# alphacep/vosk-tts

Measured on NVIDIA H100. Metric: audio samples/sec @22.05kHz, 128-phoneme utterance, higher is better.
Workload: dtype fp32 (flow/decoder convs + attention: bf16 hi+lo split x3 MMAs on wgmma, fp32 accumulate; rest fp32 FFMA)

## Files before the change

### vosk_tts_b200/csrc/conv_tc.cuh

```cuda
#pragma once
#include <type_traits>
#include <cuda.h>
#include <cuda_bf16.h>
#include <cuda_runtime.h>
#include <stdint.h>
#include "wgmma.cuh"

namespace vtts {

constexpr int TC_BM = 128;
constexpr int TC_BK = 64;
#ifndef VTTS_TC_AST64
#define VTTS_TC_AST64 3
#endif
#ifndef VTTS_TC_WST64
#define VTTS_TC_WST64 4
#endif
#ifndef VTTS_TC_AST128
#define VTTS_TC_AST128 3
#endif
#ifndef VTTS_TC_WST128
#define VTTS_TC_WST128 4
#endif
template <int BN> constexpr int tc_ast() { return BN == 64 ? VTTS_TC_AST64 : VTTS_TC_AST128; }
template <int BN> constexpr int tc_wst() { return BN == 64 ? VTTS_TC_WST64 : VTTS_TC_WST128; }
constexpr int TC_CWG = 2;
constexpr int TC_THREADS = TC_CWG * 128 + 32;
constexpr int TC_MAXP = 4;

enum : int { TCE_RELU = 1, TCE_GATE = 2 };

struct TcProblemBase {
  CUtensorMap a_hi, a_lo, w_hi, w_lo;
  __nv_bfloat16* p_mid;
  const float* bias;
  const float* cond;
  const float* res;
  float* y;
  __nv_bfloat16* p_hi;
  __nv_bfloat16* p_lo;
  int cond_ld, ldr, roff, ldy, yoff, ldp, poff;
  int Cin, Cout, k, dil, pad;
  int out_mul, out_add;
  int in_extra, out_seq_extra;
  int epi;
  float alpha, pl_slope;
  int split;
  int cl0;
};
struct TcProblem : TcProblemBase {
  CUtensorMap a_mid, w_mid;
};

struct TcBatchScalars {
  int n;
  int rmul;
  int tall;
  int a_bytes;
  int baseoff;
  int cn;
  int wpre;
  int np;
  int ast, wst;
  int dbgskip;
  int wmc;
  int persist;
  int gx, gy, gz;
  int split;
  int mixed;
  int nb;
  unsigned long long* dbg;
};
template <class PT, int MP = TC_MAXP>
struct TcBatchT : TcBatchScalars {
  PT p[MP];
};
using TcBatch = TcBatchT<TcProblem>;
template <int MP>
inline TcBatchT<TcProblemBase, MP> tc_lite(const TcBatch& tb) {
  TcBatchT<TcProblemBase, MP> l;
  static_cast<TcBatchScalars&>(l) = tb;
  for (int i = 0; i < MP; ++i) l.p[i] = tb.p[i];
  return l;
}
__device__ __forceinline__ unsigned long long gtimer() {
  unsigned long long t;
  asm volatile("mov.u64 %0, %globaltimer;" : "=l"(t));
  return t;
}
#define TC_STAMP(i) do { if (tb.dbg && blockIdx.x == 0 && blockIdx.y == 0 && blockIdx.z == 0) tb.dbg[i] = gtimer(); } while (0)

__device__ __forceinline__ void tma_load_2d(void* dst, const CUtensorMap* map, int c0, int c1, uint64_t* bar) {
  asm volatile(
      "cp.async.bulk.tensor.2d.shared::cluster.global.mbarrier::complete_tx::bytes [%0], [%1, {%3, %4}], [%2];" ::"r"(smem_u32(dst)),
      "l"(reinterpret_cast<uint64_t>(map)), "r"(smem_u32(bar)), "r"(c0), "r"(c1)
      : "memory");
}
__device__ __forceinline__ void tma_load_2d_mc(void* dst, const CUtensorMap* map, int c0, int c1, uint64_t* bar, uint16_t mask) {
  asm volatile(
      "cp.async.bulk.tensor.2d.shared::cluster.global.mbarrier::complete_tx::bytes.multicast::cluster [%0], [%1, {%3, %4}], [%2], %5;" ::"r"(
          smem_u32(dst)),
      "l"(reinterpret_cast<uint64_t>(map)), "r"(smem_u32(bar)), "r"(c0), "r"(c1), "h"(mask)
      : "memory");
}
__device__ __forceinline__ uint32_t cluster_rank() {
  uint32_t r;
  asm volatile("mov.u32 %0, %%cluster_ctarank;" : "=r"(r));
  return r;
}
__device__ __forceinline__ void mbar_arrive_remote(uint64_t* bar, uint32_t rank) {
  uint32_t ra;
  asm volatile("mapa.shared::cluster.u32 %0, %1, %2;" : "=r"(ra) : "r"(smem_u32(bar)), "r"(rank));
  asm volatile("mbarrier.arrive.release.cluster.shared::cluster.b64 _, [%0];" ::"r"(ra) : "memory");
}
__device__ __forceinline__ void tc_release(uint64_t* bar, int n) {
  if (n > 1) {
    for (int r = 0; r < n; ++r) mbar_arrive_remote(bar, (uint32_t)r);
  } else {
    mbar_arrive(bar);
  }
}


struct TcEpi {
  const float* bias;
  const float* cond;
  const float* res;
  float* y;
  __nv_bfloat16 *p_hi, *p_lo, *p_mid;
  int ldr, roff, ldy, yoff, ldp, poff;
  int ncol;
  float alpha, pl_slope;
  bool gate, relu, store;
};
template <class PT>
__device__ __forceinline__ TcEpi tc_epi(const PT& P, int b, int dbgskip) {
  TcEpi E;
  E.bias = P.bias;
  E.cond = P.cond ? P.cond + (long)b * P.cond_ld : nullptr;
  E.res = (dbgskip & 4) ? nullptr : P.res;
  E.y = P.y;
  E.p_hi = P.p_hi; E.p_lo = P.p_lo; E.p_mid = P.p_mid;
  E.ldr = P.ldr; E.roff = P.roff; E.ldy = P.ldy; E.yoff = P.yoff; E.ldp = P.ldp; E.poff = P.poff;
  E.gate = (P.epi & TCE_GATE) != 0;
  E.relu = (P.epi & TCE_RELU) != 0;
  E.ncol = E.gate ? P.Cout >> 1 : P.Cout;
  E.alpha = P.alpha; E.pl_slope = P.pl_slope;
  E.store = !(dbgskip & 1);
  return E;
}
struct TcEpiCol {
  int c, oc, nout;
  bool ok;
};
__device__ __forceinline__ TcEpiCol tc_epi_col(const TcEpi& E, int c, bool in_tile) {
  TcEpiCol k;
  k.c = c;
  k.oc = E.gate ? c >> 1 : c;
  k.ok = in_tile && k.oc < E.ncol;
  k.nout = E.gate ? 1 : min(2, E.ncol - k.oc);
  return k;
}
struct TcEpiIn {
  float b0, b1, c0, c1, r[2][2];
};
__device__ __forceinline__ TcEpiIn tc_epi_load(const TcEpi& E, const TcEpiCol& k, const long (&orow)[2], const bool (&rowok)[2]) {
  TcEpiIn in = {};
  if (!(k.ok && (rowok[0] || rowok[1]))) return in;
  const bool two = E.gate || k.nout > 1;
  in.b0 = E.bias[k.c];
  if (two) in.b1 = E.bias[k.c + 1];
  if (E.cond) {
    in.c0 = E.cond[k.c];
    if (two) in.c1 = E.cond[k.c + 1];
  }
  if (E.res) {
#pragma unroll
    for (int h = 0; h < 2; ++h) {
      if (!rowok[h]) continue;
      const float* rp = E.res + orow[h] * (long)E.ldr + E.roff + k.oc;
      if (k.nout == 2 && ((E.ldr | E.roff | k.oc) & 1) == 0) {
        const float2 q2 = *reinterpret_cast<const float2*>(rp);
        in.r[h][0] = q2.x; in.r[h][1] = q2.y;
      } else {
        in.r[h][0] = rp[0];
        if (k.nout > 1) in.r[h][1] = rp[1];
      }
    }
  }
  return in;
}
__device__ __forceinline__ void tc_epi_store(const TcEpi& E, const TcEpiCol& k, long orow, float b0, float b1, float c0, float c1,
                                             float r0, float r1, float v0, float v1) {
  const float bv0 = E.cond ? b0 + c0 : b0, bv1 = E.cond ? b1 + c1 : b1;
  float u[2];
  if (E.gate) {
    const float a = v0 + bv0, s = v1 + bv1;
    u[0] = tanhf(a) * (1.f / (1.f + expf(-s)));
    u[1] = 0.f;
  } else {
    u[0] = v0 + bv0;
    u[1] = k.nout > 1 ? v1 + bv1 : 0.f;
  }
#pragma unroll
  for (int e = 0; e < 2; ++e) {
    float q = u[e];
    if (E.relu) q = fmaxf(q, 0.f);
    u[e] = __fmul_rn(q, E.alpha);
  }
  if (E.res) {
    u[0] = __fadd_rn(u[0], r0);
    if (k.nout > 1) u[1] = __fadd_rn(u[1], r1);
  }
  if (!E.store) return;
  const int oc = k.oc, nout = k.nout;
  if (E.y) {
    float* yr = E.y + orow * (long)E.ldy + E.yoff + oc;
    if (nout == 2 && ((E.ldy | E.yoff | oc) & 1) == 0) {
      *reinterpret_cast<float2*>(yr) = make_float2(u[0], u[1]);
    } else {
      yr[0] = u[0];
      if (nout > 1) yr[1] = u[1];
    }
  }
  if (E.p_hi) {
    const long po = orow * (long)E.ldp + E.poff + oc;
    __nv_bfloat16 hb[2], mb[2], lb[2];
#pragma unroll
    for (int e = 0; e < 2; ++e) {
      float q = u[e];
      q = q > 0.f ? q : q * E.pl_slope;
      if (E.p_mid) split_bf16_3(q, hb[e], mb[e], lb[e]);
      else split_bf16(q, hb[e], lb[e]);
    }
    if (nout == 2 && ((E.ldp | E.poff | oc) & 1) == 0) {
      *reinterpret_cast<__nv_bfloat162*>(E.p_hi + po) = __halves2bfloat162(hb[0], hb[1]);
      *reinterpret_cast<__nv_bfloat162*>(E.p_lo + po) = __halves2bfloat162(lb[0], lb[1]);
      if (E.p_mid) *reinterpret_cast<__nv_bfloat162*>(E.p_mid + po) = __halves2bfloat162(mb[0], mb[1]);
    } else {
      E.p_hi[po] = hb[0]; E.p_lo[po] = lb[0];
      if (E.p_mid) E.p_mid[po] = mb[0];
      if (nout > 1) {
        E.p_hi[po + 1] = hb[1]; E.p_lo[po + 1] = lb[1];
        if (E.p_mid) E.p_mid[po + 1] = mb[1];
      }
    }
  }
}

template <int BN>
constexpr int tc_smem_bytes(int a_bytes, int np = 2, int ast = tc_ast<BN>(), int wst = tc_wst<BN>()) {
  return ast * np * a_bytes + wst * np * BN * TC_BK * 2 + 1024  + 256 ;
}
constexpr int TC_MAXST = 4;

struct TcTile {
  int pi;
  int b, co0, t0, sp;
  int s;
  int t0u;
  bool valid;
};

template <int BN, bool MIXED, class PT, int MP>
__device__ __forceinline__ void conv_tc_body(const TcBatchT<PT, MP>& tb, const int* __restrict__ lens, const int* __restrict__ offs) {
  constexpr bool HAS_MID = std::is_same<PT, TcProblem>::value;
  constexpr int B_BYTES = BN * TC_BK * 2;
  constexpr int NACC = BN / 2;
  const int TC_AST = tb.ast, TC_WST = tb.wst, NP = HAS_MID ? tb.np : 2;
  PDL_LAUNCH();
  if (threadIdx.x == 0) TC_STAMP(0);
  const int S = tb.split;
  const bool persist = tb.persist != 0;
  const int A_BYTES = tb.a_bytes;
  const bool tall = tb.tall != 0;
  const int wmc = persist ? tb.wmc : 1;
  const uint32_t wrank = wmc > 1 ? cluster_rank() : 0u;
  const int gxu = (tb.gx + wmc - 1) / wmc;
  const int ntiles = persist ? gxu * tb.gy * tb.gz : 1;
  const int tstride = persist ? (int)gridDim.x / wmc : 1;
  const int tile0 = persist ? (int)blockIdx.x / wmc : 0;
  auto decode_mixed = [&](int g) {
    const int ci = (int)blockIdx.z / S, rank = (int)blockIdx.z - ci * S;
    int pi = 0;
    while (pi + 1 < tb.n && ci >= tb.p[pi + 1].cl0) ++pi;
    const int s = tb.p[pi].split, gyp = (tb.p[pi].Cout + BN - 1) / BN;
    if (g < 0) g = rank / s;
    const int tile = (ci - tb.p[pi].cl0) * (S / s) + g;
    TcTile t;
    t.pi = pi;
    t.s = s;
    t.sp = rank % s;
    t.t0 = (tile % tb.gx) * TC_BM;
    t.t0u = t.t0;
    t.co0 = ((tile / tb.gx) % gyp) * BN;
    t.b = tile / (tb.gx * gyp);
    t.valid = t.b < tb.nb;
    return t;
  };
  auto decode = [&](int tile) {
    if constexpr (MIXED) { if (tb.mixed) return decode_mixed(-1); }
    int bx, by, bz, bxu;
    if (persist) {
      bxu = tile % gxu;
      const int r = tile / gxu;
      by = r % tb.gy;
      bz = r / tb.gy;
      bx = bxu * wmc + (int)wrank;
    } else {
      bx = blockIdx.x; by = blockIdx.y; bz = blockIdx.z;
      bxu = bx;
    }
    TcTile t;
    t.t0u = bxu * wmc * TC_BM;
    const int zi = bz / S;
    t.s = S;
    t.sp = bz - zi * S;
    t.pi = zi % tb.n;
    t.b = zi / tb.n;
    t.co0 = by * BN;
    t.t0 = bx * TC_BM;
    t.valid = t.co0 < tb.p[t.pi].Cout;
    return t;
  };

  extern __shared__ uint8_t tc_smem_raw[];
  uint8_t* smem = reinterpret_cast<uint8_t*>((reinterpret_cast<uintptr_t>(tc_smem_raw) + 1023) & ~(uintptr_t)1023);
  uint8_t* smem_w = smem + TC_AST * NP * A_BYTES;
  uint64_t* a_full = reinterpret_cast<uint64_t*>(smem_w + TC_WST * NP * B_BYTES);
  uint64_t* a_empty = a_full + TC_MAXST;
  uint64_t* w_full = a_empty + TC_MAXST;
  uint64_t* w_empty = w_full + TC_MAXST;

  const int warp = threadIdx.x >> 5, lane = threadIdx.x & 31;
  const bool producer = warp == TC_CWG * 4;
  const TcTile first = decode(tile0);
  const int cn = tb.cn;

  if (producer && lane == 0) {
    for (int s = 0; s < TC_AST; ++s) { mbar_init(&a_full[s], 1); mbar_init(&a_empty[s], (uint32_t)(cn * TC_CWG)); }
    for (int s = 0; s < TC_WST; ++s) { mbar_init(&w_full[s], 1); mbar_init(&w_empty[s], (uint32_t)(wmc * TC_CWG)); }
    asm volatile("fence.mbarrier_init.release.cluster;" ::: "memory");
    for (int q = 0; q < (persist ? tb.n : 1); ++q) {
      const PT& Q = tb.p[persist ? q : first.pi];
      asm volatile("prefetch.tensormap [%0];" ::"l"(reinterpret_cast<uint64_t>(&Q.a_hi)) : "memory");
      asm volatile("prefetch.tensormap [%0];" ::"l"(reinterpret_cast<uint64_t>(&Q.a_lo)) : "memory");
      asm volatile("prefetch.tensormap [%0];" ::"l"(reinterpret_cast<uint64_t>(&Q.w_hi)) : "memory");
      asm volatile("prefetch.tensormap [%0];" ::"l"(reinterpret_cast<uint64_t>(&Q.w_lo)) : "memory");
      if constexpr (HAS_MID) {
        if (NP == 3) {
          asm volatile("prefetch.tensormap [%0];" ::"l"(reinterpret_cast<uint64_t>(&Q.a_mid)) : "memory");
          asm volatile("prefetch.tensormap [%0];" ::"l"(reinterpret_cast<uint64_t>(&Q.w_mid)) : "memory");
        }
      }
    }
  }
  __syncthreads();
  const uint32_t crank = cn > 1 ? cluster_rank() : 0u;
  const uint16_t cmask = (uint16_t)((1u << cn) - 1u);
  if (cn > 1 || wmc > 1) cluster_sync_all();
  int w_pre = 0;
  auto issue_w = [&](const PT& P, int co0, int c, int j, int wst) {
    uint8_t* wb = smem_w + wst * NP * B_BYTES;
    mbar_expect_tx(&w_full[wst], NP * B_BYTES);
    if (wmc > 1) {
      const int half = (int)wrank * (BN / 2);
      tma_load_2d_mc(wb + half * 128, &P.w_hi, c * TC_BK, j * P.Cout + co0 + half, &w_full[wst], (uint16_t)3);
      tma_load_2d_mc(wb + B_BYTES + half * 128, &P.w_lo, c * TC_BK, j * P.Cout + co0 + half, &w_full[wst], (uint16_t)3);
      return;
    }
    tma_load_2d(wb, &P.w_hi, c * TC_BK, j * P.Cout + co0, &w_full[wst]);
    tma_load_2d(wb + B_BYTES, &P.w_lo, c * TC_BK, j * P.Cout + co0, &w_full[wst]);
    if constexpr (HAS_MID) { if (NP == 3) tma_load_2d(wb + 2 * B_BYTES, &P.w_mid, c * TC_BK, j * P.Cout + co0, &w_full[wst]); }
  };
  if (!persist && first.valid) {
    const PT& P = tb.p[first.pi];
    const int nsteps_all = (P.Cin / TC_BK) * P.k;
    const int s_beg = (int)((long)nsteps_all * first.sp / first.s), s_end = (int)((long)nsteps_all * (first.sp + 1) / first.s);
    const bool peek_active = first.t0 < lens[first.b] * tb.rmul + P.in_extra;
    w_pre = (tb.wpre && peek_active) ? min(TC_WST, s_end - s_beg) : 0;
    if (producer && lane == 0) {
      int c = s_beg / P.k, j = s_beg - c * P.k;
      for (int i = 0; i < w_pre; ++i) {
        issue_w(P, first.co0, c, j, i);
        if (++j == P.k) { j = 0; ++c; }
      }
    }
  }
  PDL_WAIT();
  if (threadIdx.x == 0) TC_STAMP(1);
  bool any_active = false;

  if (producer) {
    if (lane == 0) {
      int ast = 0, a_use = 0, wst = 0, w_use = 0;
      for (int tile = tile0; tile < ntiles; tile += tstride) {
        const TcTile T = persist ? decode(tile) : first;
        if (!T.valid) continue;
        const PT& P = tb.p[T.pi];
        const int L = lens[T.b] * tb.rmul + P.in_extra;
        if (T.t0u >= L) {
          for (int i = 0; i < w_pre; ++i) mbar_wait(&w_full[i], 0);
          continue;
        }
        any_active = true;
        const long in_base = (long)offs[T.b] * tb.rmul + (long)T.b * P.in_extra;
        const int nsteps_all = (P.Cin / TC_BK) * P.k;
        const int s_beg = (int)((long)nsteps_all * T.sp / T.s), s_end = (int)((long)nsteps_all * (T.sp + 1) / T.s);
        const int a_per = tall ? P.k : 1;
        const uint32_t a_tx = (uint32_t)NP * (uint32_t)(tall ? (TC_BM + (P.k - 1) * P.dil) : TC_BM) * 128u;
        int c = s_beg / P.k, j = s_beg - c * P.k;
        int a_cnt = 0;
        for (int s = s_beg; s < s_end; ++s) {
          const int ls = s - s_beg;
          if (a_cnt == 0) {
            if (a_use > 0) mbar_wait(&a_empty[ast], (a_use - 1) & 1);
            uint8_t* ab = smem + ast * NP * A_BYTES;
            mbar_expect_tx(&a_full[ast], a_tx);
            const int row = (int)in_base + T.t0 - P.pad + (tall ? 0 : j * P.dil);
            if (cn > 1) {
              const int slice = TC_BM / cn;
              const int soff = (int)crank * slice;
              tma_load_2d_mc(ab + soff * 128, &P.a_hi, c * TC_BK, row + soff, &a_full[ast], cmask);
              tma_load_2d_mc(ab + A_BYTES + soff * 128, &P.a_lo, c * TC_BK, row + soff, &a_full[ast], cmask);
            } else {
              tma_load_2d(ab, &P.a_hi, c * TC_BK, row, &a_full[ast]);
              tma_load_2d(ab + A_BYTES, &P.a_lo, c * TC_BK, row, &a_full[ast]);
              if constexpr (HAS_MID) { if (NP == 3) tma_load_2d(ab + 2 * A_BYTES, &P.a_mid, c * TC_BK, row, &a_full[ast]); }
            }
            if (++ast == TC_AST) { ast = 0; ++a_use; }
          }
          if (++a_cnt == a_per) a_cnt = 0;
          if (ls >= w_pre) {
            if (w_use > 0) mbar_wait(&w_empty[wst], (w_use - 1) & 1);
            issue_w(P, T.co0, c, j, wst);
          }
          if (++wst == TC_WST) { wst = 0; ++w_use; }
          if (++j == P.k) { j = 0; ++c; }
          if (ls == 0) TC_STAMP(2);
        }
        w_pre = 0;
        TC_STAMP(3);
      }
    }
    any_active = __shfl_sync(0xffffffffu, (int)any_active, 0) != 0;
  } else {
    const int wg = warp >> 2;
    const int g = lane >> 2, q4 = lane & 3;
    const int rbase = wg * 64 + (warp & 3) * 16 + g;
    const bool leader = (threadIdx.x & 127) == 0;
    int ast = 0, a_use = 0, wst = 0, w_use = 0;
    for (int tile = tile0; tile < ntiles; tile += tstride) {
      const TcTile T = persist ? decode(tile) : first;
      if (!T.valid) continue;
      const PT& P = tb.p[T.pi];
      const int L = lens[T.b] * tb.rmul + P.in_extra;
      if (T.t0u >= L) continue;
      any_active = true;
      const int nsteps_all = (P.Cin / TC_BK) * P.k;
      const int s_beg = (int)((long)nsteps_all * T.sp / T.s), s_end = (int)((long)nsteps_all * (T.sp + 1) / T.s);
      const int a_per = tall ? P.k : 1;
      float acc[NACC];
#pragma unroll
      for (int i = 0; i < NACC; ++i) acc[i] = 0.f;
      int j = s_beg % P.k;
      int a_cnt = 0;
      int prev_w = -1, prev_a = -1;
      for (int s = s_beg; s < s_end; ++s) {
        const int ls = s - s_beg;
        if (a_cnt == 0) mbar_wait(&a_full[ast], a_use & 1);
        mbar_wait(&w_full[wst], w_use & 1);
        if (ls == 0 && threadIdx.x == 0) TC_STAMP(4);
        const uint32_t abase = smem_u32(smem + ast * NP * A_BYTES) + (uint32_t)(wg * 64 * 128) + (tall ? (uint32_t)(j * P.dil) * 128u : 0u);
        const uint32_t wbase = smem_u32(smem_w + wst * NP * B_BYTES);
        const uint64_t ahi = gmma_desc_sw128(abase, tb.baseoff), alo = gmma_desc_sw128(abase + A_BYTES, tb.baseoff);
        const uint64_t bhi = gmma_desc_sw128(wbase), blo = gmma_desc_sw128(wbase + B_BYTES);
        auto mma = [&](uint64_t da, uint64_t db) {
          if constexpr (BN == 128) wgmma_ss_n128(acc, da, db);
          else wgmma_ss_n64(acc, da, db);
        };
        wgmma_fence();
        if (tb.dbgskip & 2) {
        } else if (NP == 3) {
          const uint64_t ami = gmma_desc_sw128(abase + 2 * A_BYTES, tb.baseoff), bmi = gmma_desc_sw128(wbase + 2 * B_BYTES);
#pragma unroll
          for (int kk = 0; kk < TC_BK / 16; ++kk) {
            const uint64_t adv = (uint64_t)((kk * 32) >> 4);
            mma(ahi + adv, blo + adv);
            mma(alo + adv, bhi + adv);
            mma(ami + adv, bmi + adv);
            mma(ami + adv, bhi + adv);
            mma(ahi + adv, bmi + adv);
            mma(ahi + adv, bhi + adv);
          }
        } else {
#pragma unroll
          for (int kk = 0; kk < TC_BK / 16; ++kk) {
            const uint64_t adv = (uint64_t)((kk * 32) >> 4);
            mma(alo + adv, bhi + adv);
            mma(ahi + adv, blo + adv);
            mma(ahi + adv, bhi + adv);
          }
        }
        wgmma_commit();
        wgmma_wait<1>();
        wgmma_touch<NACC>(acc);
        if (leader) {
          if (prev_w >= 0) tc_release(&w_empty[prev_w], wmc);
          if (prev_a >= 0) tc_release(&a_empty[prev_a], cn);
        }
        prev_w = wst;
        prev_a = -1;
        if (++wst == TC_WST) { wst = 0; ++w_use; }
        if (++a_cnt == a_per) {
          prev_a = ast;
          a_cnt = 0;
          if (++ast == TC_AST) { ast = 0; ++a_use; }
        }
        if (++j == P.k) j = 0;
      }
      const int W = BN / T.s, ncp = W / 8;
      const TcEpi E = tc_epi(P, T.b, tb.dbgskip);
      const int cbase = T.co0 + T.sp * W + 2 * q4;
      long orow[2];
      bool rowok[2];
      {
        const long out_base = (long)offs[T.b] * tb.rmul * P.out_mul + (long)T.b * P.out_seq_extra;
#pragma unroll
        for (int h = 0; h < 2; ++h) {
          const int t = T.t0 + rbase + 8 * h;
          rowok[h] = t < L;
          orow[h] = out_base + (long)t * P.out_mul + P.out_add;
        }
      }
      auto col = [&](int j) { return tc_epi_col(E, cbase + 8 * j, j < ncp); };
      TcEpiIn in = tc_epi_load(E, col(0), orow, rowok);
      wgmma_wait<0>();
      wgmma_touch<NACC>(acc);
      if (leader) {
        if (prev_w >= 0) tc_release(&w_empty[prev_w], wmc);
        if (prev_a >= 0) tc_release(&a_empty[prev_a], cn);
      }
      if (threadIdx.x == 0) TC_STAMP(5);
      float* stage = reinterpret_cast<float*>(smem);
      if (T.s > 1) {
        const int sp = T.sp, g0 = MIXED ? (int)blockIdx.z % S - sp : 0;
        cluster_sync_all();
#pragma unroll
        for (int jn = 0; jn < BN / 8; ++jn) {
          const int cc = jn * 8 + 2 * q4;
          const int qo = cc / W;
#pragma unroll
          for (int h = 0; h < 2; ++h) {
            uint32_t ra;
            asm volatile("mapa.shared::cluster.u32 %0, %1, %2;" : "=r"(ra) : "r"(smem_u32(stage + ((size_t)sp * TC_BM + rbase + 8 * h) * W + (cc - qo * W))), "r"(g0 + qo));
            asm volatile("st.shared::cluster.v2.f32 [%0], {%1, %2};" ::"r"(ra), "f"(acc[4 * jn + 2 * h]), "f"(acc[4 * jn + 2 * h + 1]) : "memory");
          }
        }
        cluster_sync_all();
      }
#pragma unroll 1
      for (int j = 0; j < ncp; ++j) {
        const TcEpiIn nx = tc_epi_load(E, col(j + 1), orow, rowok);
        const TcEpiCol k = col(j);
#pragma unroll 1
        for (int h = 0; h < 2; ++h) {
          if (!k.ok || !(h ? rowok[1] : rowok[0])) continue;
          float v0 = h ? acc[2] : acc[0], v1 = h ? acc[3] : acc[1];
          if (T.s > 1) {
            const float* st = stage + (size_t)(rbase + 8 * h) * W + 8 * j + 2 * q4;
            v0 = 0.f; v1 = 0.f;
#pragma unroll 1
            for (int src = 0; src < T.s; ++src) {
              const float2 p2 = *reinterpret_cast<const float2*>(st + (size_t)src * TC_BM * W);
              v0 += p2.x; v1 += p2.y;
            }
          }
          tc_epi_store(E, k, h ? orow[1] : orow[0], in.b0, in.b1, in.c0, in.c1, h ? in.r[1][0] : in.r[0][0],
                       h ? in.r[1][1] : in.r[0][1], v0, v1);
        }
#pragma unroll
        for (int i = 0; i + 4 < NACC; ++i) acc[i] = acc[i + 4];
        in = nx;
      }
    }
  }
  if (first.s > 1) {
    bool cl_active = any_active;
    if (MIXED && tb.mixed)
      for (int g = 0; g < S / first.s; ++g) {
        const TcTile u = decode_mixed(g);
        if (u.valid && u.t0 < lens[u.b] * tb.rmul + tb.p[u.pi].in_extra) cl_active = true;
      }
    if (cl_active && (producer || !any_active)) {
      __syncwarp();
      cluster_sync_all();
      cluster_sync_all();
    }
  }
  if (threadIdx.x == 0) TC_STAMP(7);
  __syncthreads();
  if (cn > 1 || wmc > 1) cluster_sync_all();
  if (threadIdx.x == 0) TC_STAMP(8);
}

template <int BN, bool DYN, int MP = TC_MAXP>
__global__ void __launch_bounds__(TC_THREADS, 1)
conv_tc_kernel(const __grid_constant__ TcBatchT<std::conditional_t<DYN, TcProblem, TcProblemBase>, MP> tb, const int* __restrict__ lens,
               const int* __restrict__ offs) {
  conv_tc_body<BN, true>(tb, lens, offs);
}
template <int BN>
__global__ void __launch_bounds__(TC_THREADS, 1)
conv_tc_persist_kernel(const __grid_constant__ TcBatch tb, const int* __restrict__ lens, const int* __restrict__ offs) {
  conv_tc_body<BN, false>(tb, lens, offs);
}

constexpr int EW_THREADS = 256;
constexpr int EW_ROWS = 16;

__global__ void __launch_bounds__(EW_THREADS)
split_planes_kernel(const float* __restrict__ x, int ldx, __nv_bfloat16* __restrict__ hi, __nv_bfloat16* __restrict__ lo,
                    int ldp, int C, float slope, int reflect, int rmul, const int* __restrict__ lens,
                    const int* __restrict__ offs) {
  PDL_LAUNCH();
  PDL_WAIT();
  const int b = blockIdx.y;
  const int Lphys = lens[b] * rmul;
  const int L = Lphys + (reflect ? 1 : 0);
  const int p0 = blockIdx.x * EW_ROWS;
  if (p0 >= L) return;
  const int nq = C >> 2;
  const int nrow = min(EW_ROWS, L - p0);
  const long base = (long)offs[b] * rmul;
  for (int u = threadIdx.x; u < nrow * nq; u += EW_THREADS) {
    const int r = u / nq, c = (u - r * nq) << 2;
    const int p = p0 + r;
    const int pr = reflect ? (p == 0 ? 1 : p - 1) : p;
    const long irow = base + pr;
    const long orow = base + (reflect ? b : 0) + p;
    const float4 v = *reinterpret_cast<const float4*>(x + irow * ldx + c);
    const float f[4] = {v.x, v.y, v.z, v.w};
    __align__(8) __nv_bfloat16 hb[4], lb[4];
#pragma unroll
    for (int i = 0; i < 4; ++i) {
      const float q = f[i] > 0.f ? f[i] : f[i] * slope;
      split_bf16(q, hb[i], lb[i]);
    }
    *reinterpret_cast<uint2*>(hi + orow * ldp + c) = *reinterpret_cast<const uint2*>(hb);
    *reinterpret_cast<uint2*>(lo + orow * ldp + c) = *reinterpret_cast<const uint2*>(lb);
  }
}

__global__ void __launch_bounds__(EW_THREADS)
mrf_mean_planes_kernel(const float* __restrict__ a, const float* __restrict__ b2, const float* __restrict__ c3, int n,
                       float* __restrict__ out, __nv_bfloat16* __restrict__ hi, __nv_bfloat16* __restrict__ lo, int C,
                       float slope, int reflect, int rmul, const int* __restrict__ lens, const int* __restrict__ offs) {
  PDL_LAUNCH();
  PDL_WAIT();
  const int b = blockIdx.y;
// ... 33 lines not shown
```

### vosk_tts_b200/csrc/engine.cu

```cuda
#include <cuda_runtime.h>
#include <stdint.h>
#include <stdio.h>
#include <string.h>
#include <stdlib.h>

#include <algorithm>
#include <chrono>
#include <condition_variable>
#include <functional>
#include <thread>
#include <initializer_list>
#include <map>
#include <mutex>
#include <sstream>
#include <string>
#include <unordered_map>
#include <vector>

#include "../../include/vtts.h"
#include "kernels.cuh"
#include "conv_tc.cuh"
#include "mas.cuh"
#include "attn_tc.cuh"
#include "vc.cuh"
// ... 1293 lines not shown
  tb.wst = np == 3 ? (BN == 128 ? 2 : 3) : (BN == 128 ? tc_wst<128>() : tc_wst<64>());
  tb.split = split;
  tb.cn = cn;
  tb.tall = tall ? 1 : 0;
  const int wmc = (big && t.tc_wmc && split == 1 && cn == 1 && np == 2 && n_sm % 2 == 0) ? 2 : 1;
  tb.baseoff = t.tc_baseoff;
  tb.dbgskip = t.tc_dbgskip;
  tb.a_bytes = (maxNR * 128 + 1023) / 1024 * 1024;
  for (size_t i = 0; i < ps.size(); ++i) {
    const TcSpec& q = ps[i];
    TcProblem& P = tb.p[i];
    const int box_rows = tall ? TC_BM + (q.k - 1) * q.dil : TC_BM / cn;
    P.a_hi = make_map(q.in.hi, q.in.C, q.in.rows, box_rows);
    P.a_lo = make_map(q.in.lo, q.in.C, q.in.rows, box_rows);
    P.w_hi = make_map(q.w.hi, q.Cin, (long)q.k * q.Cout, BN / wmc);
    P.w_lo = make_map(q.w.lo, q.Cin, (long)q.k * q.Cout, BN / wmc);
    if (np == 3) {
      P.a_mid = make_map(q.in.mid, q.in.C, q.in.rows, box_rows);
      P.w_mid = make_map(q.w.mid, q.Cin, (long)q.k * q.Cout, BN);
    }
    P.p_mid = q.out.mid;
    P.bias = q.bias;
    P.res = q.res; P.ldr = q.ldr; P.roff = q.roff;
    P.y = q.y; P.ldy = q.ldy; P.yoff = q.yoff;
    P.cond = q.cond; P.cond_ld = q.cond_ld; P.epi = q.epi;
    P.p_hi = q.out.hi; P.p_lo = q.out.lo; P.ldp = q.out.C; P.poff = q.poff;
    P.Cin = q.Cin; P.Cout = q.Cout; P.k = q.k; P.dil = q.dil; P.pad = q.pad;
    P.out_mul = q.out_mul; P.out_add = q.out_add; P.in_extra = q.in_extra; P.out_seq_extra = q.out_seq_extra;
    P.alpha = q.alpha; P.pl_slope = q.pl_slope;
    P.split = psplit[i];
    REQUIRE(q.in.C == q.Cin, VTTS_ERR_INVALID, "plane width must equal the conv input channels");
    maxCout = std::max(maxCout, q.Cout);
    maxL = std::max(maxL, maxLen * rmul + q.in_extra);
  }
  tb.n = (int)ps.size();
  tb.rmul = rmul;
  tb.dbg = tc_dbg;
  tb.nb = nB;
  dim3 grid((maxL + TC_BM - 1) / TC_BM, (maxCout + BN - 1) / BN, nB * tb.n * split);
  if (grid.x == 0) return;
  tb.wpre = one_wave ? 1 : 0;
  tb.gx = (int)grid.x; tb.gy = (int)grid.y; tb.gz = (int)grid.z;
  tb.mixed = mixed ? 1 : 0;
  if (mixed) grid = dim3(1, 1, (unsigned)tiles_all);
  tb.persist = 0;
  tb.wmc = 1;
  if (split == 1 && cn == 1 && !tb.wpre && (t.tc_persist == 2 || (t.tc_persist && (long)grid.x * grid.y * grid.z > (long)t.tc_persist_min * n_sm))) {
    tb.persist = 1;
    tb.wmc = wmc;
    grid = dim3((unsigned)n_sm, 1, 1);
  }
  REQUIRE(tb.persist || wmc == 1, VTTS_ERR_INVALID, "tensor-core conv: weight multicast planned for a launch that is not persistent");
  const bool single_wave_image = split > 1 || tb.wpre;
  const bool dyn_image = tb.np != 2 || tb.ast != (BN == 128 ? tc_ast<128>() : tc_ast<64>()) || tb.wst != (BN == 128 ? tc_wst<128>() : tc_wst<64>());
  {
    vtts_conv_report rep{};
    rep.use_tc = 1; rep.bn = BN; rep.split = split; rep.tall = tb.tall; rep.cn = cn; rep.wmc = tb.wmc; rep.persist = tb.persist; rep.np = tb.np;
    rep.ast = tb.ast; rep.wst = tb.wst; rep.image = single_wave_image ? (dyn_image ? 1 : 0) : 2;
    rep.grid_x = (int)grid.x; rep.grid_y = (int)grid.y; rep.grid_z = (int)grid.z;
    for (size_t p = 0; p < ps.size(); ++p) rep.psplit[p] = psplit[p];
    note_conv(rep);
  }
  if (profiling) {
    if (tc_prof_used + 2 > tc_prof_ev.size()) {
      tc_prof_ev.resize(tc_prof_used + 2);
      CK(cudaEventCreate(tc_prof_ev[tc_prof_used].out()));
      CK(cudaEventCreate(tc_prof_ev[tc_prof_used + 1].out()));
    }
    for (const TcSpec& q : ps)
      for (int b = 0; b < nB; ++b)
        tc_prof_flops += 2.0 * ((double)r.real[b] * rmul + q.in_extra) * q.Cout * q.Cin * q.k;
    ++tc_prof_launches;
    CK(cudaEventRecord(tc_prof_ev[tc_prof_used], stream));
  }
  {
    cudaLaunchConfig_t lc;
    memset(&lc, 0, sizeof(lc));
    lc.gridDim = grid; lc.blockDim = dim3(TC_THREADS); lc.stream = stream;
    lc.dynamicSmemBytes = BN == 128 ? tc_smem_bytes<128>(tb.a_bytes, tb.np, tb.ast, tb.wst) : tc_smem_bytes<64>(tb.a_bytes, tb.np, tb.ast, tb.wst);
    REQUIRE(lc.dynamicSmemBytes <= 227 * 1024, VTTS_ERR_INVALID, "tensor-core conv: shared-memory budget exceeded");
    cudaLaunchAttribute at[2];
    int na = 0;
    if (cn > 1 || split > 1 || tb.wmc > 1) {
      at[na].id = cudaLaunchAttributeClusterDimension;
      at[na].val.clusterDim.x = tb.wmc; at[na].val.clusterDim.y = cn; at[na].val.clusterDim.z = split;
      ++na;
    }
    if (use_pdl) {
      at[na].id = cudaLaunchAttributeProgrammaticStreamSerialization;
      at[na].val.programmaticStreamSerializationAllowed = 1;
      ++na;
    }
    lc.attrs = at; lc.numAttrs = na;
    if (single_wave_image) {
      if (dyn_image) {
        if (BN == 128) CK(cudaLaunchKernelEx(&lc, conv_tc_kernel<128, true>, tb, r.lens, r.offs));
        else CK(cudaLaunchKernelEx(&lc, conv_tc_kernel<64, true>, tb, r.lens, r.offs));
      } else {
        const auto tl = tc_lite<TC_MAXP>(tb);
        if (BN == 128) CK(cudaLaunchKernelEx(&lc, conv_tc_kernel<128, false, TC_MAXP>, tl, r.lens, r.offs));
        else CK(cudaLaunchKernelEx(&lc, conv_tc_kernel<64, false, TC_MAXP>, tl, r.lens, r.offs));
      }
    } else {
      if (BN == 128) CK(cudaLaunchKernelEx(&lc, conv_tc_persist_kernel<128>, tb, r.lens, r.offs));
      else CK(cudaLaunchKernelEx(&lc, conv_tc_persist_kernel<64>, tb, r.lens, r.offs));
    }
  }
  CK(cudaGetLastError());
  if (profiling) {
    CK(cudaEventRecord(tc_prof_ev[tc_prof_used + 1], stream));
    tc_prof_used += 2;
  }
  ++launches;
}

bool vtts_engine::attn_tc_ok(const EncLayerW& L, int Hc, const Tuning& t) const {
  const int dk = Hc / L.heads;
  return t.attn_tc_mode > 0 && L.rk_hi != nullptr && dk % 32 == 0 && dk <= 128 && 2 * cfg.window_size + 1 <= ATC_RS && (3 * Hc) % 8 == 0;
}
bool vtts_engine::attn_use_tc(const EncLayerW& L, int Hc, const Rows& r) const {
  const Tuning& t = r.tune;
  if (!attn_tc_ok(L, Hc, t)) return false;
  if (t.attn_tc_mode >= 2) return true;
  return !((t.attn_rows == 0 || t.attn_rows == 1) && attn_split_fits(L, Hc, r));
}

bool vtts_engine::attn_split_fits(const EncLayerW& L, int Hc, const Rows& r) const {
  const int dk = Hc / L.heads, nrel = 2 * cfg.window_size + 1;
  long ctas = 0;
  for (int b = 0; b < r.n; ++b) ctas += (long)((r.sized[b] + ATS_ROWS - 1) / ATS_ROWS) * L.heads;
  const int mt = (r.maxLen + AT_KT - 1) / AT_KT;
  return r.tune.attn_split && mt <= ATS_MAXT && ctas <= n_sm && dk % 32 == 0 && dk <= 128 &&
         (long)attn_split_smem_floats(dk, nrel, mt) * (long)sizeof(float) <= ATS_SMEM_MAX;
// ... 3463 lines not shown
  }
  const int lo = keep_off[0], hi = keep_off[B - 1] + keep_len[B - 1];
  for (int& o : keep_off) o -= lo;
  read_clips(read_back(h, same ? h->d_rsin : h->d_rsout, (size_t)(hi - lo), 0, (size_t)lo), keep_off.data(), keep_len, 1, out, out_ld);
  for (int b = 0; b < B; ++b) out_lengths[b] = keep_len[b];
}

static void impl_synthesize_dev(vtts_handle h, const float* d_noise_z, int z_ld, float* d_wav, int64_t wav_ld) {
  REQUIRE(h->have_durations, VTTS_ERR_STATE, "vtts_synthesize_dev called without vtts_durations_dev");
  REQUIRE((int64_t)h->real_maxFrm * h->hop <= wav_ld, VTTS_ERR_CAPACITY, "wav_ld is smaller than hop * max(y_lengths)");
  REQUIRE(!d_noise_z || z_ld >= h->real_maxFrm, VTTS_ERR_CAPACITY, "noise_z has fewer columns than max(y_lengths)");
  h->run_graphed({vtts_engine::TAG_PHASE2_DEV, h->B, h->maxFrm, h->Tfrm, z_ld, (long long)(uintptr_t)d_noise_z}, [&] { h->phase2(d_noise_z, z_ld, true); });
  for (int b = 0; b < h->B; ++b)
    CK(cudaMemcpyAsync(d_wav + (size_t)b * wav_ld, h->d_wav.p + (size_t)h->h_frm_off[b] * h->hop,
                       (size_t)h->h_frm_len[b] * h->hop * sizeof(float), cudaMemcpyDeviceToDevice, h->stream));
  CK(cudaEventRecord(h->ev[7], h->stream));
  CK(cudaStreamSynchronize(h->stream));
  collect_timings(h);
  h->have_durations = false;
}

}

extern "C" {

int vtts_create(const vtts_config* cfg, const float* blob, size_t blob_floats, const char* manifest, int blob_is_device,
                int device, vtts_handle* out) {
  if (!cfg || !blob || !manifest || !out) return VTTS_ERR_INVALID;
  *out = nullptr;
  vtts_engine* h = new vtts_engine();
  for (int k = 0; k < vtts_engine::STG_KINDS; ++k) { h->stg[k].e = h; h->stg[k].readback = k >= vtts_engine::STG_OUT; }
  h->cfg = *cfg;
  h->device = device;
  *out = h;
  return guarded(h, [&] {
    REQUIRE(cfg->precision >= 0 && cfg->precision <= 3, VTTS_ERR_INVALID, "unknown precision mode");
    if (cfg->precision >= 1) {
      void* fn = nullptr;
      cudaDriverEntryPointQueryResult qres;
      CK(cudaGetDriverEntryPoint("cuTensorMapEncodeTiled", &fn, cudaEnableDefault, &qres));
      REQUIRE(fn != nullptr && qres == cudaDriverEntryPointSuccess, VTTS_ERR_CUDA, "cuTensorMapEncodeTiled is not available");
      h->encode_tiled = reinterpret_cast<vtts_engine::EncodeFn>(fn);
      CK(cudaFuncSetAttribute(conv_tc_persist_kernel<64>, cudaFuncAttributeMaxDynamicSharedMemorySize, 227 * 1024));
      CK(cudaFuncSetAttribute(conv_tc_persist_kernel<128>, cudaFuncAttributeMaxDynamicSharedMemorySize, 227 * 1024));
      CK(cudaFuncSetAttribute(conv_tc_kernel<64, false>, cudaFuncAttributeMaxDynamicSharedMemorySize, 227 * 1024));
      CK(cudaFuncSetAttribute(conv_tc_kernel<128, false>, cudaFuncAttributeMaxDynamicSharedMemorySize, 227 * 1024));
      CK(cudaFuncSetAttribute(conv_tc_kernel<64, true>, cudaFuncAttributeMaxDynamicSharedMemorySize, 227 * 1024));
      CK(cudaFuncSetAttribute(conv_tc_kernel<128, true>, cudaFuncAttributeMaxDynamicSharedMemorySize, 227 * 1024));
      for (int wi = 0; wi < 2; ++wi)
        for (int si = 0; si < 3; ++si) {
          const int S = 2 << si;
          cudaLaunchConfig_t lc;
          memset(&lc, 0, sizeof(lc));
          lc.gridDim = dim3(1, 1, S * 64); lc.blockDim = dim3(TC_THREADS);
          lc.dynamicSmemBytes = wi ? tc_smem_bytes<128>(16 * 1024) : tc_smem_bytes<64>(16 * 1024);
          cudaLaunchAttribute at[1];
          at[0].id = cudaLaunchAttributeClusterDimension;
          at[0].val.clusterDim.x = 1; at[0].val.clusterDim.y = 1; at[0].val.clusterDim.z = S;
          lc.attrs = at; lc.numAttrs = 1;
          int nc = 0;
          cudaError_t e = wi ? cudaOccupancyMaxActiveClusters(&nc, conv_tc_kernel<128, false>, &lc) : cudaOccupancyMaxActiveClusters(&nc, conv_tc_kernel<64, false>, &lc);
          if (e != cudaSuccess) { nc = 0; cudaGetLastError(); }
          h->tc_cluster_cap[wi][si] = nc;
        }
      if (getenv("VTTS_VERBOSE"))
        fprintf(stderr, "[vtts] co-resident conv_tc clusters: BN64 %d/%d/%d  BN128 %d/%d/%d (S=2/4/8)\n", h->tc_cluster_cap[0][0], h->tc_cluster_cap[0][1],
                h->tc_cluster_cap[0][2], h->tc_cluster_cap[1][0], h->tc_cluster_cap[1][1], h->tc_cluster_cap[1][2]);
    }
    CK(cudaDeviceGetAttribute(&h->n_sm, cudaDevAttrMultiProcessorCount, device));
    CK(cudaStreamCreateWithFlags(h->stream.out(), cudaStreamNonBlocking));
    for (auto& st : h->side) CK(cudaStreamCreateWithFlags(st.out(), cudaStreamNonBlocking));
    CK(cudaEventCreateWithFlags(h->ev_fork.out(), cudaEventDisableTiming));
    for (auto& e : h->ev_join) CK(cudaEventCreateWithFlags(e.out(), cudaEventDisableTiming));
    for (auto& e : h->ev) CK(cudaEventCreate(e.out()));
    h->blob_floats = blob_floats;
    CK(h->d_blob.alloc(blob_floats));
    CK(cudaMemcpyAsync(h->d_blob.p, blob, blob_floats * sizeof(float), blob_is_device ? cudaMemcpyDeviceToDevice : cudaMemcpyHostToDevice, h->stream));
    std::istringstream is(manifest);
    std::string name;
    unsigned long long off, n;
    while (is >> name >> off >> n) {
      REQUIRE(off + n <= blob_floats, VTTS_ERR_WEIGHTS, "manifest entry exceeds the blob");
      h->tensors[name] = Tensor{h->d_blob.p + off, (size_t)n};
    }
    h->tune = Tuning::from_env();
    if (const char* e = getenv("VTTS_MRF_BRANCH")) h->mrf_branch = atoi(e);
    if (const char* e = getenv("VTTS_MRF_HEAVY_FIRST")) h->mrf_heavy_first = atoi(e);
    if (const char* e = getenv("VTTS_PDL")) h->use_pdl = atoi(e) != 0;
    if (const char* e = getenv("VTTS_NO_POLL")) h->use_poll = atoi(e) == 0;
    if (const char* e = getenv("VTTS_NO_GRAPHS")) h->use_graphs = atoi(e) == 0;
    if (const char* e = getenv("VTTS_BUCKETS")) h->use_buckets = atoi(e) != 0;
    if (const char* e = getenv("VTTS_SPEC")) h->use_spec = atoi(e) != 0;
    if (const char* e = getenv("VTTS_SPEC_MARGIN")) h->spec_margin = (float)atof(e);
    if (const char* e = getenv("VTTS_CAPTURE_FIRST")) h->capture_on_first = atoi(e) != 0;
    if (const char* e = getenv("VTTS_PREFETCH")) h->use_prefetch = atoi(e) != 0;
    REQUIRE(cfg->model_family >= VTTS_FAMILY_VITS2 && cfg->model_family <= VTTS_FAMILY_SOVITS, VTTS_ERR_INVALID, "unknown model family");
    if (cfg->model_family == VTTS_FAMILY_QUICKVC) h->bind_quickvc();
    else if (cfg->model_family == VTTS_FAMILY_T2S) h->bind_t2s();
    else if (cfg->model_family == VTTS_FAMILY_SOVITS) h->bind_sovits();
    else if (cfg->model_family == VTTS_FAMILY_STABLETTS) {
      h->bind_stabletts();
      h->bind_bert();
    }
    else h->bind_weights();
    h->build_prefetch_list();
    CK(cudaMemsetAsync(h->ensure(h->d_done_ctr, 4), 0, 4 * sizeof(int), h->stream));
    CK(cudaFuncSetAttribute(dds_layer_kernel<DDS_TT>, cudaFuncAttributeMaxDynamicSharedMemorySize, 160 * 1024));
// ... 1647 lines not shown
    CK(cudaMemcpy(dl.p, hl, 8, cudaMemcpyHostToDevice)); CK(cudaMemcpy(dof.p, ho, 8, cudaMemcpyHostToDevice));
    const Rows r{dl.p, dof.p, 1, rows, {rows}, {rows}, h->tune};
    CK(y.alloc((size_t)rows * Cout)); CK(bias.alloc(ldw)); CK(cudaMemset(bias.p, 0, (size_t)ldw * 4));
    if (is_tc) {
      CK(ph.alloc((size_t)rows * Cin)); CK(pl.alloc((size_t)rows * Cin));
      CK(wh.alloc((size_t)k * Cout * Cin)); CK(wl.alloc((size_t)k * Cout * Cin));
      CK(cudaMemset(ph.p, 0, (size_t)rows * Cin * 2)); CK(cudaMemset(pl.p, 0, (size_t)rows * Cin * 2));
      CK(cudaMemset(wh.p, 0, (size_t)k * Cout * Cin * 2)); CK(cudaMemset(wl.p, 0, (size_t)k * Cout * Cin * 2));
    } else {
      CK(x.alloc((size_t)rows * Cin)); CK(w.alloc((size_t)k * Cin * ldw));
      CK(cudaMemset(x.p, 0, (size_t)rows * Cin * 4)); CK(cudaMemset(w.p, 0, (size_t)k * Cin * ldw * 4));
    }
    auto once = [&] {
      if (is_tc) {
        TcSpec q;
        q.in.hi = ph.p; q.in.lo = pl.p; q.in.C = Cin; q.in.rows = rows;
        q.w.hi = wh.p; q.w.lo = wl.p; q.bias = bias.p; q.Cin = Cin; q.Cout = Cout; q.k = k; q.dil = dil; q.pad = dil * (k - 1) / 2;
        q.y = y.p; q.ldy = Cout;
        h->launch_tc({q}, 1, r);
      } else {
        ConvW W; W.w = w.p; W.b = bias.p; W.Cin = Cin; W.Cout = Cout; W.k = k; W.ldw = ldw;
        h->launch_conv({mk(W, x.p, Cin, 0, y.p, Cout, 0, dil, dil * (k - 1) / 2)}, 1, r);
      }
    };
    h->profiling = false;
    for (int i = 0; i < 3; ++i) once();
    Event e0, e1;
    CK(cudaEventCreate(e0.out())); CK(cudaEventCreate(e1.out()));
    Graph graph;
    GraphExec gexec;
    CK(cudaStreamBeginCapture(h->stream, cudaStreamCaptureModeThreadLocal));
    for (int i = 0; i < iters; ++i) once();
    CK(cudaStreamEndCapture(h->stream, graph.out()));
    CK(cudaGraphInstantiate(gexec.out(), graph, 0));
    CK(cudaGraphLaunch(gexec, h->stream));
    CK(cudaStreamSynchronize(h->stream));
    CK(cudaEventRecord(e0, h->stream));
    CK(cudaGraphLaunch(gexec, h->stream));
    CK(cudaEventRecord(e1, h->stream));
    CK(cudaStreamSynchronize(h->stream));
    if (is_tc && getenv("VTTS_TC_STAMPS")) {
      Buf<unsigned long long> d;
      CK(d.alloc(16)); CK(cudaMemset(d.p, 0, 16 * 8));
      h->tc_dbg = d.p;
      Event a0, a1; CK(cudaEventCreate(a0.out())); CK(cudaEventCreate(a1.out()));
      CK(cudaEventRecord(a0, h->stream));
      once();
      CK(cudaEventRecord(a1, h->stream));
      CK(cudaStreamSynchronize(h->stream));
      h->tc_dbg = nullptr;
      unsigned long long st[16];
      CK(cudaMemcpy(st, d.p, sizeof(st), cudaMemcpyDeviceToHost));
      float one = 0.f; CK(cudaEventElapsedTime(&one, a0, a1));
      fprintf(stderr, "[tc stamps %s] event %.2f us | entry->setup %.2f | ->first TMA issued %.2f | ->all TMA issued %.2f | ->first full %.2f | ->mma issued %.2f | ->acc ready %.2f | ->epi done %.2f | ->sync %.2f (us since entry)\n",
              what, one * 1e3, (st[1] - st[0]) / 1e3, (st[2] - st[0]) / 1e3, (st[3] - st[0]) / 1e3, (st[4] - st[0]) / 1e3,
              (st[5] - st[0]) / 1e3, (st[6] - st[0]) / 1e3, (st[7] - st[0]) / 1e3, (st[8] - st[0]) / 1e3);
    }
    float ms = 0.f;
    CK(cudaEventElapsedTime(&ms, e0, e1));
    result = ms / iters;
  });
  return rc == VTTS_OK ? result : (float)rc;
}

}
```

Before: 21.69 million.

## Stage epilogue bias/cond/residual into shared memory via dedicated cp.async warp

Adds a second auxiliary warp to the split-K/single-wave conv kernel that prefetches the bias, conditioning and residual tiles into swizzled shared memory with cp.async while the MMA mainloop runs. Consumers wait on an mbarrier and read the epilogue operands from shared memory instead of issuing global loads after the accumulators are ready. The goal is to take epilogue global-load latency off the critical path of these latency-bound launches. In exchange it uses extra shared memory, which can force smaller operand ring depths, and an extra warp per block.

```diff
diff --git a/vosk_tts_b200/csrc/conv_tc.cuh b/vosk_tts_b200/csrc/conv_tc.cuh
--- a/vosk_tts_b200/csrc/conv_tc.cuh
+++ b/vosk_tts_b200/csrc/conv_tc.cuh
@@ -26,6 +26,7 @@
 template <int BN> constexpr int tc_wst() { return BN == 64 ? VTTS_TC_WST64 : VTTS_TC_WST128; }
 constexpr int TC_CWG = 2;
 constexpr int TC_THREADS = TC_CWG * 128 + 32;
+constexpr int TC_THREADS_SW = TC_THREADS + 32;
 constexpr int TC_MAXP = 4;
 
 enum : int { TCE_RELU = 1, TCE_GATE = 2 };
@@ -121,6 +122,17 @@
   }
 }
 
+__device__ __forceinline__ void cp_async4(void* dst, const void* src) {
+  asm volatile("cp.async.ca.shared.global [%0], [%1], 4;" ::"r"(smem_u32(dst)), "l"(__cvta_generic_to_global(src)) : "memory");
+}
+__device__ __forceinline__ void cp_async16(void* dst, const void* src) {
+  asm volatile("cp.async.cg.shared.global [%0], [%1], 16;" ::"r"(smem_u32(dst)), "l"(__cvta_generic_to_global(src)) : "memory");
+}
+__device__ __forceinline__ void cp_async_arrive(uint64_t* bar) {
+  asm volatile("cp.async.mbarrier.arrive.noinc.shared::cta.b64 [%0];" ::"r"(smem_u32(bar)) : "memory");
+}
+__device__ __forceinline__ void cp_async_wait_all() { asm volatile("cp.async.wait_all;" ::: "memory"); }
+
 
 struct TcEpi {
   const float* bias;
@@ -190,6 +202,64 @@
   }
   return in;
 }
+
+__host__ __device__ constexpr int tc_epi_rs(int wr) { return wr < 32 ? 32 : wr; }
+__host__ __device__ constexpr int tc_epi_bytes(int w, int wr, bool res) { return 8 * w + (res ? TC_BM * tc_epi_rs(wr) * 4 : 0); }
+struct TcStage {
+  float *bias, *cond, *res;
+  int rs, sm, ss;
+};
+__device__ __forceinline__ TcStage tc_stage(float* base, int w, bool gate) {
+  TcStage s;
+  s.bias = base;
+  s.cond = base + w;
+  s.res = base + 2 * w;
+  s.rs = tc_epi_rs(gate ? w >> 1 : w);
+  s.sm = gate ? 7 : 3;
+  s.ss = gate ? 2 : 3;
+  return s;
+}
+__device__ __forceinline__ void tc_stage_copy(float* dst, int ldd, int sm, int ss, const float* src, long lds, int rows, int n, int l) {
+  const int nq = (n + 3) >> 2;
+  const bool v16 = ((__cvta_generic_to_global(src) | (size_t)(lds * 4)) & 15) == 0;
+  if (v16 && nq > 0 && (n & 3) == 0 && 32 % nq == 0) {
+    const int rstep = 32 / nq, c = 4 * (l % nq);
+    for (int r = l / nq; r < rows; r += rstep) cp_async16(dst + r * ldd + (c ^ ((r & sm) << ss)), src + r * lds + c);
+    return;
+  }
+  for (int u = l; u < rows * nq; u += 32) {
+    const int r = u / nq, c = 4 * (u - r * nq);
+    const float* s = src + r * lds + c;
+    float* d = dst + r * ldd + (c ^ ((r & sm) << ss));
+    if (v16 && c + 4 <= n) {
+      cp_async16(d, s);
+    } else {
+      for (int e = 0; e < 4 && c + e < n; ++e) cp_async4(d + e, s + e);
+    }
+  }
+}
+__device__ __forceinline__ TcEpiIn tc_epi_staged(const TcEpi& E, const TcStage& S, int cl, int r0) {
+  TcEpiIn in;
+  const float2 b2 = *reinterpret_cast<const float2*>(S.bias + cl);
+  in.b0 = b2.x; in.b1 = b2.y;
+  const float2 c2 = *reinterpret_cast<const float2*>(S.cond + cl);
+  in.c0 = c2.x; in.c1 = c2.y;
+  if (E.res) {
+    const int oi = E.gate ? cl >> 1 : cl;
+#pragma unroll
+    for (int h = 0; h < 2; ++h) {
+      const int r = r0 + 8 * h;
+      const float* rp = S.res + r * S.rs + (oi ^ ((r & S.sm) << S.ss));
+      if (E.gate) {
+        in.r[h][0] = rp[0];
+      } else {
+        const float2 q2 = *reinterpret_cast<const float2*>(rp);
+        in.r[h][0] = q2.x; in.r[h][1] = q2.y;
+      }
+    }
+  }
+  return in;
+}
 __device__ __forceinline__ void tc_epi_store(const TcEpi& E, const TcEpiCol& k, long orow, float b0, float b1, float c0, float c1,
                                              float r0, float r1, float v0, float v1) {
   const float bv0 = E.cond ? b0 + c0 : b0, bv1 = E.cond ? b1 + c1 : b1;
@@ -249,8 +319,8 @@
 }
 
 template <int BN>
-constexpr int tc_smem_bytes(int a_bytes, int np = 2, int ast = tc_ast<BN>(), int wst = tc_wst<BN>()) {
-  return ast * np * a_bytes + wst * np * BN * TC_BK * 2 + 1024  + 256 ;
+constexpr int tc_smem_bytes(int a_bytes, int np = 2, int ast = tc_ast<BN>(), int wst = tc_wst<BN>(), int epi = 0) {
+  return ast * np * a_bytes + wst * np * BN * TC_BK * 2 + 1024  + 256  + epi ;
 }
 constexpr int TC_MAXST = 4;
 
@@ -264,6 +334,7 @@
 
 template <int BN, bool MIXED, class PT, int MP>
 __device__ __forceinline__ void conv_tc_body(const TcBatchT<PT, MP>& tb, const int* __restrict__ lens, const int* __restrict__ offs) {
+  constexpr bool STAGE = MIXED;
   constexpr bool HAS_MID = std::is_same<PT, TcProblem>::value;
   constexpr int B_BYTES = BN * TC_BK * 2;
   constexpr int NACC = BN / 2;
@@ -331,15 +402,21 @@
   uint64_t* a_empty = a_full + TC_MAXST;
   uint64_t* w_full = a_empty + TC_MAXST;
   uint64_t* w_empty = w_full + TC_MAXST;
+  uint64_t* e_full = w_empty + TC_MAXST;
 
   const int warp = threadIdx.x >> 5, lane = threadIdx.x & 31;
   const bool producer = warp == TC_CWG * 4;
+  const bool stager = STAGE && warp == TC_CWG * 4 + 1;
   const TcTile first = decode(tile0);
   const int cn = tb.cn;
+  const int scol = first.co0 + first.sp * (BN / first.s);
+  const TcStage stg = tc_stage(reinterpret_cast<float*>(reinterpret_cast<uint8_t*>(a_full) + 256), BN / first.s,
+                               (tb.p[first.pi].epi & TCE_GATE) != 0);
 
   if (producer && lane == 0) {
     for (int s = 0; s < TC_AST; ++s) { mbar_init(&a_full[s], 1); mbar_init(&a_empty[s], (uint32_t)(cn * TC_CWG)); }
     for (int s = 0; s < TC_WST; ++s) { mbar_init(&w_full[s], 1); mbar_init(&w_empty[s], (uint32_t)(wmc * TC_CWG)); }
+    if constexpr (STAGE) mbar_init(e_full, 32);
     asm volatile("fence.mbarrier_init.release.cluster;" ::: "memory");
     for (int q = 0; q < (persist ? tb.n : 1); ++q) {
       const PT& Q = tb.p[persist ? q : first.pi];
@@ -386,6 +463,7 @@
         if (++j == P.k) { j = 0; ++c; }
       }
     }
+    if (stager && peek_active) tc_stage_copy(stg.bias, 0, 0, 0, P.bias + scol, 0, 1, min(BN / first.s, P.Cout - scol), lane);
   }
   PDL_WAIT();
   if (threadIdx.x == 0) TC_STAMP(1);
@@ -444,6 +522,25 @@
       }
     }
     any_active = __shfl_sync(0xffffffffu, (int)any_active, 0) != 0;
+  } else if (stager) {
+    if (first.valid) {
+      const PT& P = tb.p[first.pi];
+      const int L = lens[first.b] * tb.rmul + P.in_extra;
+      if (first.t0 < L) {
+        any_active = true;
+        const int W = BN / first.s;
+        if (P.cond) tc_stage_copy(stg.cond, 0, 0, 0, P.cond + (long)first.b * P.cond_ld + scol, 0, 1, min(W, P.Cout - scol), lane);
+        if (P.res && !(tb.dbgskip & 4)) {
+          const bool gate = (P.epi & TCE_GATE) != 0;
+          const int ncol = gate ? P.Cout >> 1 : P.Cout, oc0 = gate ? scol >> 1 : scol;
+          const long row0 = (long)offs[first.b] * tb.rmul * P.out_mul + (long)first.b * P.out_seq_extra + (long)first.t0 * P.out_mul + P.out_add;
+          tc_stage_copy(stg.res, stg.rs, stg.sm, stg.ss, P.res + row0 * P.ldr + P.roff + oc0, (long)P.out_mul * P.ldr,
+                        min(TC_BM, L - first.t0), min(gate ? W >> 1 : W, ncol - oc0), lane);
+        }
+      }
+    }
+    cp_async_arrive(e_full);
+    cp_async_wait_all();
   } else {
     const int wg = warp >> 2;
     const int g = lane >> 2, q4 = lane & 3;
@@ -534,7 +631,8 @@
         }
       }
       auto col = [&](int j) { return tc_epi_col(E, cbase + 8 * j, j < ncp); };
-      TcEpiIn in = tc_epi_load(E, col(0), orow, rowok);
+      TcEpiIn in = {};
+      if constexpr (!STAGE) in = tc_epi_load(E, col(0), orow, rowok);
       wgmma_wait<0>();
       wgmma_touch<NACC>(acc);
       if (leader) {
@@ -542,6 +640,10 @@
         if (prev_a >= 0) tc_release(&a_empty[prev_a], cn);
       }
       if (threadIdx.x == 0) TC_STAMP(5);
+      if constexpr (STAGE) {
+        mbar_wait(e_full, 0);
+        if (threadIdx.x == 0) TC_STAMP(6);
+      }
       float* stage = reinterpret_cast<float*>(smem);
       if (T.s > 1) {
         const int sp = T.sp, g0 = MIXED ? (int)blockIdx.z % S - sp : 0;
@@ -561,7 +663,9 @@
       }
 #pragma unroll 1
       for (int j = 0; j < ncp; ++j) {
-        const TcEpiIn nx = tc_epi_load(E, col(j + 1), orow, rowok);
+        TcEpiIn nx;
+        if constexpr (STAGE) in = tc_epi_staged(E, stg, 8 * j + 2 * q4, rbase);
+        else nx = tc_epi_load(E, col(j + 1), orow, rowok);
         const TcEpiCol k = col(j);
 #pragma unroll 1
         for (int h = 0; h < 2; ++h) {
@@ -581,7 +685,7 @@
         }
 #pragma unroll
         for (int i = 0; i + 4 < NACC; ++i) acc[i] = acc[i + 4];
-        in = nx;
+        if constexpr (!STAGE) in = nx;
       }
     }
   }
@@ -592,7 +696,7 @@
         const TcTile u = decode_mixed(g);
         if (u.valid && u.t0 < lens[u.b] * tb.rmul + tb.p[u.pi].in_extra) cl_active = true;
       }
-    if (cl_active && (producer || !any_active)) {
+    if (cl_active && (producer || stager || !any_active)) {
       __syncwarp();
       cluster_sync_all();
       cluster_sync_all();
@@ -605,7 +709,7 @@
 }
 
 template <int BN, bool DYN, int MP = TC_MAXP>
-__global__ void __launch_bounds__(TC_THREADS, 1)
+__global__ void __launch_bounds__(TC_THREADS_SW, 1)
 conv_tc_kernel(const __grid_constant__ TcBatchT<std::conditional_t<DYN, TcProblem, TcProblemBase>, MP> tb, const int* __restrict__ lens,
                const int* __restrict__ offs) {
   conv_tc_body<BN, true>(tb, lens, offs);
diff --git a/vosk_tts_b200/csrc/engine.cu b/vosk_tts_b200/csrc/engine.cu
--- a/vosk_tts_b200/csrc/engine.cu
+++ b/vosk_tts_b200/csrc/engine.cu
@@ -1369,7 +1369,22 @@
   }
   REQUIRE(tb.persist || wmc == 1, VTTS_ERR_INVALID, "tensor-core conv: weight multicast planned for a launch that is not persistent");
   const bool single_wave_image = split > 1 || tb.wpre;
-  const bool dyn_image = tb.np != 2 || tb.ast != (BN == 128 ? tc_ast<128>() : tc_ast<64>()) || tb.wst != (BN == 128 ? tc_wst<128>() : tc_wst<64>());
+  int epi_bytes = 0;
+  if (single_wave_image)
+    for (size_t p = 0; p < ps.size(); ++p) {
+      const int w = BN / psplit[p];
+      const bool res = ps[p].res && !(tb.dbgskip & 4);
+      epi_bytes = std::max(epi_bytes, tc_epi_bytes(w, (ps[p].epi & TCE_GATE) ? w / 2 : w, res));
+    }
+  auto smem_bytes = [&] {
+    return BN == 128 ? tc_smem_bytes<128>(tb.a_bytes, tb.np, tb.ast, tb.wst, epi_bytes) : tc_smem_bytes<64>(tb.a_bytes, tb.np, tb.ast, tb.wst, epi_bytes);
+  };
+  while (smem_bytes() > 227 * 1024 && (tb.ast > 2 || tb.wst > 2)) {
+    if (tb.wst > tb.ast) --tb.wst;
+    else --tb.ast;
+  }
+  REQUIRE(smem_bytes() <= 227 * 1024, VTTS_ERR_INVALID, "tensor-core conv: operand rings and staged epilogue operands exceed 227 KB of shared memory");
+  const bool dyn_image = tb.np != 2 || tb.tall;
   {
     vtts_conv_report rep{};
     rep.use_tc = 1; rep.bn = BN; rep.split = split; rep.tall = tb.tall; rep.cn = cn; rep.wmc = tb.wmc; rep.persist = tb.persist; rep.np = tb.np;
@@ -1393,9 +1408,8 @@
   {
     cudaLaunchConfig_t lc;
     memset(&lc, 0, sizeof(lc));
-    lc.gridDim = grid; lc.blockDim = dim3(TC_THREADS); lc.stream = stream;
-    lc.dynamicSmemBytes = BN == 128 ? tc_smem_bytes<128>(tb.a_bytes, tb.np, tb.ast, tb.wst) : tc_smem_bytes<64>(tb.a_bytes, tb.np, tb.ast, tb.wst);
-    REQUIRE(lc.dynamicSmemBytes <= 227 * 1024, VTTS_ERR_INVALID, "tensor-core conv: shared-memory budget exceeded");
+    lc.gridDim = grid; lc.blockDim = dim3(single_wave_image ? TC_THREADS_SW : TC_THREADS); lc.stream = stream;
+    lc.dynamicSmemBytes = smem_bytes();
     cudaLaunchAttribute at[2];
     int na = 0;
     if (cn > 1 || split > 1 || tb.wmc > 1) {
@@ -4965,7 +4979,7 @@
           const int S = 2 << si;
           cudaLaunchConfig_t lc;
           memset(&lc, 0, sizeof(lc));
-          lc.gridDim = dim3(1, 1, S * 64); lc.blockDim = dim3(TC_THREADS);
+          lc.gridDim = dim3(1, 1, S * 64); lc.blockDim = dim3(TC_THREADS_SW);
           lc.dynamicSmemBytes = wi ? tc_smem_bytes<128>(16 * 1024) : tc_smem_bytes<64>(16 * 1024);
           cudaLaunchAttribute at[1];
           at[0].id = cudaLaunchAttributeClusterDimension;
@@ -6719,7 +6733,7 @@
       unsigned long long st[16];
       CK(cudaMemcpy(st, d.p, sizeof(st), cudaMemcpyDeviceToHost));
       float one = 0.f; CK(cudaEventElapsedTime(&one, a0, a1));
-      fprintf(stderr, "[tc stamps %s] event %.2f us | entry->setup %.2f | ->first TMA issued %.2f | ->all TMA issued %.2f | ->first full %.2f | ->mma issued %.2f | ->acc ready %.2f | ->epi done %.2f | ->sync %.2f (us since entry)\n",
+      fprintf(stderr, "[tc stamps %s] event %.2f us | entry->setup %.2f | ->first TMA issued %.2f | ->all TMA issued %.2f | ->first full %.2f | ->mma issued %.2f | ->epi operands landed %.2f | ->epi done %.2f | ->sync %.2f (us since entry)\n",
               what, one * 1e3, (st[1] - st[0]) / 1e3, (st[2] - st[0]) / 1e3, (st[3] - st[0]) / 1e3, (st[4] - st[0]) / 1e3,
               (st[5] - st[0]) / 1e3, (st[6] - st[0]) / 1e3, (st[7] - st[0]) / 1e3, (st[8] - st[0]) / 1e3);
     }
```

Result: no change. 21.74 million, median of 6 (+0.2%).
